# lyuchenyang/Macaw-LLM

Measured on NVIDIA H100. Metric: multimodal prefill tokens/sec (img+audio+text->LLaMA), higher is better.
Workload: dtype fp16

## Files before the change

### include/macaw_b200.h

```cpp
#ifndef MACAW_B200_H_
#define MACAW_B200_H_

#include <stdint.h>

#ifdef __cplusplus
extern "C" {
#endif

const char* mm_last_error(void);
int32_t mm_abi_version(void);
const char* mm_build_hash(void);
int64_t mm_launch_count(void);
void mm_launch_count_reset(void);
void mm_set_act_format(int32_t f16);
int32_t mm_get_act_format(void);

enum {
  MM_ACT_NONE = 0,
  MM_ACT_GELU = 1,
  MM_ACT_QUICK_GELU = 2,
  MM_ACT_SILU = 3
};
enum {
  MM_EPI_STD = 0,
  MM_EPI_SWIGLU = 1,
  MM_EPI_ROPE = 2
};

typedef struct mm_gemm_args {
  int32_t M, N, K, batch, batch2;
  const void* A;
  int64_t lda, a_bs, a_bs2;
  const void* B;
  int64_t ldb, b_bs, b_bs2;
  int32_t b_mn_major;
  void* C;
  int64_t ldc, c_bs, c_bs2;
  int32_t c_fp32;
  int32_t epi;
  int32_t act;
  float alpha;
  const void* bias;
  int64_t bias_bs;
  const float* row_scale;
  const void* residual;
  int64_t ldr, r_bs, r_bs2;
  int32_t res_row_mod;
  const float* rope_cos;
  const float* rope_sin;
  int32_t rope_T, rope_cols;
  const int32_t* rope_pos;
  int32_t c_trans;
  int32_t a_fp16, b_fp16;
  int32_t c_fp16;
  const float* bias_rs;
  const void* bias2;
  const float* bias2_rs;
  int32_t a_mn_major;
  float* sumsq_out;
  const float* rs_sumsq;
  int32_t rs_parts;
  float rs_eps;
  void* sk_workspace;
  int64_t sk_workspace_bytes;
} mm_gemm_args;

int32_t mm_gemm_fwd(const mm_gemm_args* args, void* stream);
enum {
  MM_GEMM_KERNEL_CONSUMER_EPILOGUE = 0,
  MM_GEMM_KERNEL_EPILOGUE_WARPGROUP = 1,
  MM_GEMM_KERNEL_TILE_PAIRS = 2
};
typedef struct mm_gemm_schedule {
  int32_t block_n;
  int32_t kernel;
  int32_t m_tiles, n_tiles, k_blocks;
  int64_t units;
  int32_t workers;
  int32_t grid;
  int32_t threads;
  int32_t waves;
  int32_t group_m;
  int32_t streamk_tiles;
  int32_t smem_bytes;
  int32_t vectorised_epilogue;
} mm_gemm_schedule;
int32_t mm_gemm_plan(const mm_gemm_args* args, mm_gemm_schedule* plan);
int32_t mm_gemm_streamk_mode(int32_t mode);
int32_t mm_gemm_overlap_mode(int32_t mode);
int64_t mm_gemm_streamk_workspace_bytes(void);

int32_t mm_splitk_reduce(const float* partial, int32_t splits, int32_t M, int32_t N, const void* bias, void* out,
                         int64_t ldo, int32_t out_fp16, void* stream);

typedef struct mm_attn_args {
  const void *q, *k, *v;
  void* out;
  int32_t B, H, Tq, Tk, head_dim;
  int64_t q_bs, q_ts, q_hs;
  int64_t k_bs, k_ts, k_hs;
  int64_t v_bs, v_ts, v_hs;
  int64_t o_bs, o_ts, o_hs;
  const int32_t* key_mask;
  int32_t causal;
  float scale;
  const int32_t* tk_dev;
} mm_attn_args;
int32_t mm_attn_fwd(const mm_attn_args* args, void* stream);

int32_t mm_rmsnorm_fwd(const void* x, const void* w, void* y, int32_t rows, int32_t cols, float eps, void* stream);
int32_t mm_rms_rstd(const void* x, float* rstd, int32_t rows, int32_t cols, float eps, void* stream);
int32_t mm_layernorm_fwd(const void* x, int64_t ldx, const void* w, const void* b, void* y, int64_t ldy, int32_t rows,
                         int32_t cols, float eps, void* stream);

int32_t mm_embed_gather(const void* table, int32_t vocab, int32_t dim, const int64_t* ids, int64_t n_ids, void* out,
                        int64_t ldo, void* stream);
int32_t mm_splice_prefix(const void* text, const void* prefix, void* dst, int32_t B, int32_t L, int32_t n_prefix,
                         int32_t E, const int64_t* mask_in, int64_t* mask_out, const int64_t* labels_in,
                         int64_t* labels_out, void* stream);
int32_t mm_patchify(const void* images, int32_t B, int32_t C, int32_t H, int32_t W, int32_t patch, void* out,
                    int64_t ldo, void* stream);
int32_t mm_transpose_pad(const void* x, int32_t B, int32_t C, int32_t T, int32_t pad, void* out, void* stream);
int32_t mm_add_rows(const void* x, int64_t ldx, const void* add, int64_t lda, int32_t add_rows, void* y, int64_t ldy,
                    int32_t rows, int32_t cols, void* stream);
int32_t mm_cast_bf16_f16(const void* x, int64_t ldx, void* y, int64_t ldy, int32_t rows, int32_t cols, void* stream);
int32_t mm_copy_rows(const void* x, int64_t ldx, void* y, int64_t ldy, int32_t rows, int32_t cols, void* stream);

typedef struct mm_align_args {
  const void* table;
  int32_t V, E;
  int64_t ldt;
  const void* qt;
  int32_t R;
  int64_t ldq;
  const float* row_bias;
  const float* extra;
  int64_t stat_stride;
  void* out;
  int64_t ldo;
  float* p_sum_real;
  float* p_extra;
  void* P;
  int64_t ldp;
  void* workspace;
  int32_t mode;
  float* inv_l;
} mm_align_args;
int32_t mm_align_fwd(const mm_align_args* args, void* stream);
int64_t mm_align_workspace_bytes(int32_t R, int32_t V);

int32_t mm_kv_append(const void* qkv, int64_t ld_qkv, int32_t B, int32_t T_new, int32_t E, void* cache, int32_t Tmax,
                     int32_t t0, const int32_t* t0_dev, void* stream);
int32_t mm_argmax_rows(const void* logits, int64_t ld, int32_t rows, int32_t V, int64_t* out, void* stream);
int32_t mm_sample_rows(const void* logits, int64_t ld, int32_t rows, int32_t V, uint32_t* seen, float repetition_penalty,
                       float temperature, int32_t top_k, float top_p, int32_t do_sample, const uint64_t* seed_dev,
                       const int32_t* step_dev, int64_t* out, void* stream);
enum { MM_THIN_RES = 0, MM_THIN_SWIGLU = 1, MM_THIN_QKV = 2 };
typedef struct mm_thin_args {
  const float* part;
  int32_t splits, N, M, ldp, mode;
  const float* row_scale;
  const float* rs_sumsq;
  int32_t rs_parts, rs_K;
  float rs_eps;
  const void* residual;
  int64_t ldr;
  void* out;
  int64_t ldo;
  float* sumsq_out;
  const float* rope_cos;
  const float* rope_sin;
  const int32_t* pos_dev;
  int32_t E;
  void* cache;
  int32_t Tmax, t0;
  const int32_t* t0_dev;
} mm_thin_args;
int32_t mm_thin_fused(const mm_thin_args* args, void* stream);
int32_t mm_rope_rows(void* x, int64_t ld, int32_t rows, int32_t rot_cols, const float* cos_t, const float* sin_t,
                     int32_t rope_T, const int32_t* pos_dev, void* stream);

int32_t mm_ce_loss(const void* logits, const int64_t* labels, int32_t B, int32_t T, int32_t V, float* loss_sum,
                   int32_t* n_valid, void* stream);

int32_t mm_rmsnorm_bwd_parts(int32_t rows);
int32_t mm_rmsnorm_bwd(const void* dy, const void* x, const float* rstd, const void* g, const void* dres, void* dx,
                       float* dg, float* dg_partials, int32_t rows, int32_t cols, void* stream);
int32_t mm_swiglu_fwd(const void* gate, const void* up, void* h, int64_t n, void* stream);
int32_t mm_swiglu_bwd(const void* dh, const void* gate, const void* up, void* dgate, void* dup, int64_t n, void* stream);
int32_t mm_attn_softmax_bwd(const float* S, const float* dP, void* P, void* dS, int32_t B, int32_t H, int32_t Tq,
                            int32_t Tk, int64_t ld, float scale, int32_t causal, const int32_t* key_mask, float p_drop,
                            const uint64_t* seed_dev, uint32_t sid, void* stream);
int32_t mm_attn_softmax_fwd(const float* S, void* P, int32_t B, int32_t H, int32_t Tq, int32_t Tk, int64_t ld, float scale,
                            int32_t causal, const int32_t* key_mask, float p_drop, const uint64_t* seed_dev, uint32_t sid,
                            void* stream);
int32_t mm_align_dropout_fwd(const void* P_unnorm_f16, void* Pm_f16, int64_t ldp, const float* inv_l, const float* p_extra,
                             float* rs, float* p_sum_real_d, float* p_extra_d, int32_t R, int32_t V, float p_drop,
                             const uint64_t* seed_dev, uint32_t sid, void* stream);
int32_t mm_dropout_mask(float* out, int64_t ld, int32_t rows, int32_t cols, float p_drop, const uint64_t* seed_dev,
                        uint32_t sid, void* stream);
int32_t mm_ce_bwd(const void* logits, const int64_t* labels, void* dlogits, int32_t B, int32_t T, int32_t V,
                  const int32_t* n_valid, float grad_scale, const float* grad_scale_dev, void* stream);
int32_t mm_embed_scatter_add(const void* dx, int64_t ldx, const int64_t* ids, int64_t n, int32_t dim, int32_t vocab,
                             void* dtable, void* stream);
int32_t mm_colsum(const void* x, int64_t ldx, int32_t rows, int32_t cols, float* out, void* stream);
int32_t mm_adamw(void* p, const void* g, float* master, float* m, float* v, int64_t n, float lr, float beta1, float beta2,
                 float eps, float weight_decay, int32_t step, const int32_t* step_dev, float grad_scale,
                 const float* grad_mult_dev, const int32_t* skip_dev, const float* lr_dev, void* stream);
int32_t mm_adamw_host(void* p, const void* g, float* master, float* m, float* v, int64_t n, float lr, float beta1,
                      float beta2, float eps, float weight_decay, int32_t step, const int32_t* step_dev, float grad_scale,
                      const float* grad_mult_dev, const int32_t* skip_dev, const float* lr_dev, void* stream);
int32_t mm_host_alloc(int64_t bytes, void** host_ptr, void** dev_ptr);
int32_t mm_host_free(void* host_ptr);

int32_t mm_grad_sumsq_parts(int64_t n);
int32_t mm_grad_sumsq(const void* g, int64_t n, int32_t fp16, float* out, float* partials, void* stream);
typedef struct mm_loss_scale_state {
  float scale;
  float inv_scale;
  int32_t cur_iter;
  int32_t last_overflow_iter;
  int32_t cur_hysteresis;
  int32_t skip;
  float grad_mult;
  int32_t skipped;
  int32_t step;
  float grad_norm;
  int32_t reserved[2];
} mm_loss_scale_state;
int32_t mm_loss_scale_update(mm_loss_scale_state* state, float* sumsq, float max_norm, int32_t dynamic, int32_t window,
                             int32_t hysteresis, float min_scale, void* stream);

int32_t mm_lr_schedule(const int32_t* step_dev, double base_lr, int32_t kind, int32_t warmup_steps, int32_t training_steps,
                       float* lr_out, void* stream);

int32_t mm_align_softmax_bwd(const float* G, int64_t ldg, const void* P_unnorm_f16, int64_t ldp, const float* inv_l,
                             const float* d_p_sum_real, const float* p_extra, const float* d_p_extra, float gscale,
                             void* P_bf16, void* dS_bf16, int64_t ldo, float* dstats, int32_t R, int32_t V, float p_drop,
                             const uint64_t* seed_dev, uint32_t sid, void* stream);
int32_t mm_head_weighted_colsum(const void* x, int64_t ldx, int32_t x_fp16, const float* w, int64_t w_stride, int32_t Nq,
                                int32_t E, int32_t head_dim, float* out, void* stream);
int32_t mm_window_gather_add(const void* dwin, int32_t B, int32_t N, int32_t C, int32_t Lq, int32_t kk, int32_t ss,
                             void* dfeats, void* stream);
int32_t mm_cast_f16_bf16(const void* x, int64_t ldx, void* y, int64_t ldy, int32_t rows, int32_t cols, void* stream);

#define MM_LORA_MAX 3
typedef struct mm_lora_args {
  int32_t n, M, K, N, r;
  float scaling, p_drop;
  const uint64_t* seed_dev;
  uint32_t sid[MM_LORA_MAX];
  const void* x;
  int64_t ldx;
  const void* A[MM_LORA_MAX];
  const void* B[MM_LORA_MAX];
  float* u[MM_LORA_MAX];
  void* y[MM_LORA_MAX];
  int64_t ldy;
  const float* rope_cos;
  const float* rope_sin;
  int32_t rope_T;
  float* g[MM_LORA_MAX];
  void* dA[MM_LORA_MAX];
  void* dB[MM_LORA_MAX];
  int32_t accumulate[MM_LORA_MAX];
  void* dx;
  int64_t lddx;
  float* workspace;
  int64_t workspace_bytes;
} mm_lora_args;
int32_t mm_lora_down(const mm_lora_args* args, void* stream);
int32_t mm_lora_up(const mm_lora_args* args, void* stream);
int32_t mm_lora_bwd_dy(const mm_lora_args* args, void* stream);
int32_t mm_lora_bwd_x(const mm_lora_args* args, void* stream);
int64_t mm_lora_workspace_bytes(const mm_lora_args* args, int32_t entry);

int32_t mm_nccl_unique_id(void* out128);
int32_t mm_nccl_init(const void* id128, int32_t world, int32_t rank);
int32_t mm_nccl_allreduce(void* buf, int64_t count, int32_t dtype, int32_t average, void* stream);
int32_t mm_nccl_destroy(void);

typedef struct mm_image_args {
  const void* src;
  int64_t ld;
  int32_t row0, n_rows;
  int32_t out_h, out_w;
  const int32_t* bounds_h;
  const int32_t* kk_h;
  int32_t ksize_h;
  const int32_t* bounds_v;
  const int32_t* kk_v;
  int32_t ksize_v;
  float mean[3], std[3];
  void* tmp;
  void* out;
  int32_t out_fp32;
  void* out_u8;
} mm_image_args;
int32_t mm_image_preprocess(const mm_image_args* args, void* stream);
int32_t mm_log_mel(const float* pcm, int32_t n_samples, const float* basisT, const float* mel, float* logspec,
                   void* max_scratch, void* out, int32_t out_fp32, void* stream);

#ifdef __cplusplus
}
#endif
#endif
```

### macaw-llm_b200/_lib.py

```python
from __future__ import annotations

import ctypes as C
import os

HERE = os.path.dirname(os.path.abspath(__file__))
LIB_PATH = os.path.join(HERE, "libmacaw_b200.so")

c_i32, c_i64, c_f32, c_vp, c_u32 = C.c_int32, C.c_int64, C.c_float, C.c_void_p, C.c_uint32


class GemmArgs(C.Structure):

    _fields_ = [
        ("M", c_i32), ("N", c_i32), ("K", c_i32), ("batch", c_i32), ("batch2", c_i32),
        ("A", c_vp), ("lda", c_i64), ("a_bs", c_i64), ("a_bs2", c_i64),
        ("B", c_vp), ("ldb", c_i64), ("b_bs", c_i64), ("b_bs2", c_i64), ("b_mn_major", c_i32),
        ("C", c_vp), ("ldc", c_i64), ("c_bs", c_i64), ("c_bs2", c_i64), ("c_fp32", c_i32),
        ("epi", c_i32), ("act", c_i32), ("alpha", c_f32),
        ("bias", c_vp), ("bias_bs", c_i64),
        ("row_scale", c_vp),
        ("residual", c_vp), ("ldr", c_i64), ("r_bs", c_i64), ("r_bs2", c_i64), ("res_row_mod", c_i32),
        ("rope_cos", c_vp), ("rope_sin", c_vp), ("rope_T", c_i32), ("rope_cols", c_i32), ("rope_pos", c_vp), ("c_trans", c_i32),
        ("a_fp16", c_i32), ("b_fp16", c_i32), ("c_fp16", c_i32),
        ("bias_rs", c_vp), ("bias2", c_vp), ("bias2_rs", c_vp), ("a_mn_major", c_i32),
        ("sumsq_out", c_vp), ("rs_sumsq", c_vp), ("rs_parts", c_i32), ("rs_eps", c_f32),
        ("sk_workspace", c_vp), ("sk_workspace_bytes", c_i64),
    ]


class GemmPlan(C.Structure):

    _fields_ = [("block_n", c_i32), ("kernel", c_i32), ("m_tiles", c_i32), ("n_tiles", c_i32), ("k_blocks", c_i32),
                ("units", c_i64), ("workers", c_i32), ("grid", c_i32), ("threads", c_i32), ("waves", c_i32),
                ("group_m", c_i32), ("streamk_tiles", c_i32), ("smem_bytes", c_i32), ("vectorised_epilogue", c_i32)]


class ThinArgs(C.Structure):
    _fields_ = [("part", c_vp), ("splits", c_i32), ("N", c_i32), ("M", c_i32), ("ldp", c_i32), ("mode", c_i32),
                ("row_scale", c_vp), ("rs_sumsq", c_vp), ("rs_parts", c_i32), ("rs_K", c_i32), ("rs_eps", c_f32),
                ("residual", c_vp), ("ldr", c_i64), ("out", c_vp), ("ldo", c_i64), ("sumsq_out", c_vp),
                ("rope_cos", c_vp), ("rope_sin", c_vp), ("pos_dev", c_vp), ("E", c_i32), ("cache", c_vp),
                ("Tmax", c_i32), ("t0", c_i32), ("t0_dev", c_vp)]


class AttnArgs(C.Structure):

    _fields_ = [
        ("q", c_vp), ("k", c_vp), ("v", c_vp), ("out", c_vp),
        ("B", c_i32), ("H", c_i32), ("Tq", c_i32), ("Tk", c_i32), ("head_dim", c_i32),
        ("q_bs", c_i64), ("q_ts", c_i64), ("q_hs", c_i64),
        ("k_bs", c_i64), ("k_ts", c_i64), ("k_hs", c_i64),
        ("v_bs", c_i64), ("v_ts", c_i64), ("v_hs", c_i64),
        ("o_bs", c_i64), ("o_ts", c_i64), ("o_hs", c_i64),
        ("key_mask", c_vp), ("causal", c_i32), ("scale", c_f32), ("tk_dev", c_vp),
    ]


class AlignArgs(C.Structure):

    _fields_ = [
        ("table", c_vp), ("V", c_i32), ("E", c_i32), ("ldt", c_i64),
        ("qt", c_vp), ("R", c_i32), ("ldq", c_i64),
        ("row_bias", c_vp), ("extra", c_vp), ("stat_stride", c_i64),
        ("out", c_vp), ("ldo", c_i64), ("p_sum_real", c_vp), ("p_extra", c_vp),
        ("P", c_vp), ("ldp", c_i64), ("workspace", c_vp), ("mode", c_i32), ("inv_l", c_vp),
    ]


LORA_MAX = 3


class LoraArgs(C.Structure):

    _fields_ = [
        ("n", c_i32), ("M", c_i32), ("K", c_i32), ("N", c_i32), ("r", c_i32), ("scaling", c_f32), ("p_drop", c_f32),
        ("seed_dev", c_vp), ("sid", c_u32 * LORA_MAX), ("x", c_vp), ("ldx", c_i64), ("A", c_vp * LORA_MAX),
        ("B", c_vp * LORA_MAX), ("u", c_vp * LORA_MAX), ("y", c_vp * LORA_MAX), ("ldy", c_i64), ("rope_cos", c_vp),
        ("rope_sin", c_vp), ("rope_T", c_i32), ("g", c_vp * LORA_MAX), ("dA", c_vp * LORA_MAX), ("dB", c_vp * LORA_MAX),
        ("accumulate", c_i32 * LORA_MAX), ("dx", c_vp), ("lddx", c_i64), ("workspace", c_vp), ("workspace_bytes", c_i64),
    ]


class LossScaleState(C.Structure):

    _fields_ = [("scale", c_f32), ("inv_scale", c_f32), ("cur_iter", c_i32), ("last_overflow_iter", c_i32),
                ("cur_hysteresis", c_i32), ("skip", c_i32), ("grad_mult", c_f32), ("skipped", c_i32), ("step", c_i32),
                ("grad_norm", c_f32), ("reserved", c_i32 * 2)]


class ImageArgs(C.Structure):

    _fields_ = [
        ("src", c_vp), ("ld", c_i64), ("row0", c_i32), ("n_rows", c_i32), ("out_h", c_i32), ("out_w", c_i32),
        ("bounds_h", c_vp), ("kk_h", c_vp), ("ksize_h", c_i32), ("bounds_v", c_vp), ("kk_v", c_vp), ("ksize_v", c_i32),
        ("mean", c_f32 * 3), ("std", c_f32 * 3), ("tmp", c_vp), ("out", c_vp), ("out_fp32", c_i32), ("out_u8", c_vp),
    ]


SIGNATURES = {
    "mm_last_error": (C.c_char_p, []),
    "mm_abi_version": (c_i32, []),
    "mm_build_hash": (C.c_char_p, []),
    "mm_launch_count": (c_i64, []),
    "mm_launch_count_reset": (None, []),
    "mm_set_act_format": (None, [c_i32]),
    "mm_get_act_format": (c_i32, []),
    "mm_gemm_fwd": (c_i32, [C.POINTER(GemmArgs), c_vp]),
    "mm_gemm_plan": (c_i32, [C.POINTER(GemmArgs), C.POINTER(GemmPlan)]),
    "mm_splitk_reduce": (c_i32, [c_vp, c_i32, c_i32, c_i32, c_vp, c_vp, c_i64, c_i32, c_vp]),
    "mm_attn_fwd": (c_i32, [C.POINTER(AttnArgs), c_vp]),
    "mm_rmsnorm_fwd": (c_i32, [c_vp, c_vp, c_vp, c_i32, c_i32, c_f32, c_vp]),
    "mm_rms_rstd": (c_i32, [c_vp, c_vp, c_i32, c_i32, c_f32, c_vp]),
    "mm_layernorm_fwd": (c_i32, [c_vp, c_i64, c_vp, c_vp, c_vp, c_i64, c_i32, c_i32, c_f32, c_vp]),
    "mm_embed_gather": (c_i32, [c_vp, c_i32, c_i32, c_vp, c_i64, c_vp, c_i64, c_vp]),
    "mm_splice_prefix": (c_i32, [c_vp, c_vp, c_vp, c_i32, c_i32, c_i32, c_i32, c_vp, c_vp, c_vp, c_vp, c_vp]),
    "mm_patchify": (c_i32, [c_vp, c_i32, c_i32, c_i32, c_i32, c_i32, c_vp, c_i64, c_vp]),
    "mm_transpose_pad": (c_i32, [c_vp, c_i32, c_i32, c_i32, c_i32, c_vp, c_vp]),
    "mm_add_rows": (c_i32, [c_vp, c_i64, c_vp, c_i64, c_i32, c_vp, c_i64, c_i32, c_i32, c_vp]),
    "mm_cast_bf16_f16": (c_i32, [c_vp, c_i64, c_vp, c_i64, c_i32, c_i32, c_vp]),
    "mm_copy_rows": (c_i32, [c_vp, c_i64, c_vp, c_i64, c_i32, c_i32, c_vp]),
    "mm_align_fwd": (c_i32, [C.POINTER(AlignArgs), c_vp]),
    "mm_align_workspace_bytes": (c_i64, [c_i32, c_i32]),
    "mm_kv_append": (c_i32, [c_vp, c_i64, c_i32, c_i32, c_i32, c_vp, c_i32, c_i32, c_vp, c_vp]),
    "mm_gemm_streamk_workspace_bytes": (c_i64, []),
    "mm_gemm_streamk_mode": (c_i32, [c_i32]),
    "mm_gemm_overlap_mode": (c_i32, [c_i32]),
    "mm_thin_fused": (c_i32, [C.POINTER(ThinArgs), c_vp]),
    "mm_argmax_rows": (c_i32, [c_vp, c_i64, c_i32, c_i32, c_vp, c_vp]),
    "mm_sample_rows": (c_i32, [c_vp, c_i64, c_i32, c_i32, c_vp, c_f32, c_f32, c_i32, c_f32, c_i32, c_vp, c_vp, c_vp, c_vp]),
    "mm_rope_rows": (c_i32, [c_vp, c_i64, c_i32, c_i32, c_vp, c_vp, c_i32, c_vp, c_vp]),
    "mm_rmsnorm_bwd": (c_i32, [c_vp, c_vp, c_vp, c_vp, c_vp, c_vp, c_vp, c_vp, c_i32, c_i32, c_vp]),
    "mm_rmsnorm_bwd_parts": (c_i32, [c_i32]),
    "mm_swiglu_fwd": (c_i32, [c_vp, c_vp, c_vp, c_i64, c_vp]),
    "mm_swiglu_bwd": (c_i32, [c_vp, c_vp, c_vp, c_vp, c_vp, c_i64, c_vp]),
    "mm_attn_softmax_bwd": (c_i32, [c_vp, c_vp, c_vp, c_vp, c_i32, c_i32, c_i32, c_i32, c_i64, c_f32, c_i32, c_vp, c_f32, c_vp,
                                    c_u32, c_vp]),
    "mm_attn_softmax_fwd": (c_i32, [c_vp, c_vp, c_i32, c_i32, c_i32, c_i32, c_i64, c_f32, c_i32, c_vp, c_f32, c_vp, c_u32, c_vp]),
    "mm_align_dropout_fwd": (c_i32, [c_vp, c_vp, c_i64, c_vp, c_vp, c_vp, c_vp, c_vp, c_i32, c_i32, c_f32, c_vp, c_u32, c_vp]),
    "mm_dropout_mask": (c_i32, [c_vp, c_i64, c_i32, c_i32, c_f32, c_vp, c_u32, c_vp]),
    "mm_ce_bwd": (c_i32, [c_vp, c_vp, c_vp, c_i32, c_i32, c_i32, c_vp, c_f32, c_vp, c_vp]),
    "mm_embed_scatter_add": (c_i32, [c_vp, c_i64, c_vp, c_i64, c_i32, c_i32, c_vp, c_vp]),
    "mm_colsum": (c_i32, [c_vp, c_i64, c_i32, c_i32, c_vp, c_vp]),
    "mm_adamw": (c_i32, [c_vp, c_vp, c_vp, c_vp, c_vp, c_i64, c_f32, c_f32, c_f32, c_f32, c_f32, c_i32, c_vp, c_f32, c_vp,
                         c_vp, c_vp, c_vp]),
    "mm_adamw_host": (c_i32, [c_vp, c_vp, c_vp, c_vp, c_vp, c_i64, c_f32, c_f32, c_f32, c_f32, c_f32, c_i32, c_vp, c_f32,
                              c_vp, c_vp, c_vp, c_vp]),
    "mm_lr_schedule": (c_i32, [c_vp, C.c_double, c_i32, c_i32, c_i32, c_vp, c_vp]),
    "mm_host_alloc": (c_i32, [c_i64, C.POINTER(c_vp), C.POINTER(c_vp)]),
    "mm_host_free": (c_i32, [c_vp]),
    "mm_grad_sumsq_parts": (c_i32, [c_i64]),
    "mm_grad_sumsq": (c_i32, [c_vp, c_i64, c_i32, c_vp, c_vp, c_vp]),
    "mm_loss_scale_update": (c_i32, [c_vp, c_vp, c_f32, c_i32, c_i32, c_i32, c_f32, c_vp]),
    "mm_image_preprocess": (c_i32, [C.POINTER(ImageArgs), c_vp]),
    "mm_log_mel": (c_i32, [c_vp, c_i32, c_vp, c_vp, c_vp, c_vp, c_vp, c_i32, c_vp]),
    "mm_align_softmax_bwd": (c_i32, [c_vp, c_i64, c_vp, c_i64, c_vp, c_vp, c_vp, c_vp, c_f32, c_vp, c_vp, c_i64, c_vp, c_i32,
                                     c_i32, c_f32, c_vp, c_u32, c_vp]),
    "mm_head_weighted_colsum": (c_i32, [c_vp, c_i64, c_i32, c_vp, c_i64, c_i32, c_i32, c_i32, c_vp, c_vp]),
    "mm_window_gather_add": (c_i32, [c_vp, c_i32, c_i32, c_i32, c_i32, c_i32, c_i32, c_vp, c_vp]),
    "mm_cast_f16_bf16": (c_i32, [c_vp, c_i64, c_vp, c_i64, c_i32, c_i32, c_vp]),
    "mm_nccl_unique_id": (c_i32, [c_vp]),
    "mm_nccl_init": (c_i32, [c_vp, c_i32, c_i32]),
    "mm_nccl_allreduce": (c_i32, [c_vp, c_i64, c_i32, c_i32, c_vp]),
    "mm_nccl_destroy": (c_i32, []),
    "mm_ce_loss": (c_i32, [c_vp, c_vp, c_i32, c_i32, c_i32, c_vp, c_vp, c_vp]),
    "mm_lora_down": (c_i32, [C.POINTER(LoraArgs), c_vp]),
    "mm_lora_up": (c_i32, [C.POINTER(LoraArgs), c_vp]),
    "mm_lora_bwd_dy": (c_i32, [C.POINTER(LoraArgs), c_vp]),
    "mm_lora_bwd_x": (c_i32, [C.POINTER(LoraArgs), c_vp]),
    "mm_lora_workspace_bytes": (c_i64, [C.POINTER(LoraArgs), c_i32]),
}

NULLABLE_BEFORE_STREAM = {"mm_adamw": 1, "mm_adamw_host": 1}

_lib = None
ABI_VERSION = 8


class _NullableBeforeStream:

    def __init__(self, fn, n_opt: int):
        self._fn, self._n_opt = fn, n_opt

    def __call__(self, *args):
        n = len(self._fn.argtypes)
        if n - self._n_opt <= len(args) < n:
            args = args[:-1] + (None,) * (n - len(args)) + args[-1:]
        return self._fn(*args)

    def __getattr__(self, name):
        return getattr(self._fn, name)


def load(build_if_missing: bool = True) -> C.CDLL:
    global _lib
    if _lib is not None:
        return _lib
    import importlib.util

    spec = importlib.util.spec_from_file_location("_macaw_b200_build", os.path.join(HERE, "build.py"))
    mod = importlib.util.module_from_spec(spec)
    spec.loader.exec_module(mod)
    want = mod.source_hash()
    if not os.path.exists(LIB_PATH) or mod.built_hash() != want:
        if not build_if_missing:
            raise RuntimeError(f"{LIB_PATH} is missing or older than csrc/; run `python macaw-llm_b200/build.py`")
        mod.build()
    lib = C.CDLL(LIB_PATH)
    for name, (res, args) in SIGNATURES.items():
        fn = getattr(lib, name)
        fn.restype = res
        fn.argtypes = args
        if name in NULLABLE_BEFORE_STREAM:
            setattr(lib, name, _NullableBeforeStream(fn, NULLABLE_BEFORE_STREAM[name]))
    got = lib.mm_build_hash().decode()
    if got != want or lib.mm_abi_version() != ABI_VERSION:
        raise RuntimeError(f"libmacaw_b200.so was built from other sources (library {got}, csrc {want}; ABI "
                           f"{lib.mm_abi_version()} vs {ABI_VERSION}): rebuild with `python macaw-llm_b200/build.py --force`")
    _lib = lib
    return lib


def last_error() -> str:
    return load().mm_last_error().decode("utf-8", "replace")
```

### macaw-llm_b200/csrc/attn_wgmma.cu

```cuda
#include "common.cuh"
#include "ptx.cuh"
#include "../../include/macaw_b200.h"

namespace mm {

struct FaParams {
  bf16* out;
  int B, H, Tq, Tk;
  long long o_bs, o_ts, o_hs;
  const int* key_mask;
  const int* tk_dev;
  int causal;
  float scale_log2;
  int hd;
};

constexpr int kFaMQ = 128;
constexpr int kFaKT = 64;
constexpr int kFaThreads = 288;

template <int HD>
__host__ __device__ constexpr size_t fa_smem_bytes() {
  return 1024 + (size_t)(HD / 64) * 16384 + 4 * (size_t)(HD / 64) * kFaKT * 128 + 256;
}

template <bool F16>
__device__ __forceinline__ void wgmma_s(float (&d)[kFaKT / 2], uint64_t a, uint64_t b, uint32_t acc) {
  wgmma_ss_n64<F16, 0, 0>(d, a, b, acc);
}
template <int HD, bool F16>
__device__ __forceinline__ void wgmma_pv(float (&d)[HD / 2], const uint32_t (&a)[4], uint64_t b) {
  if constexpr (HD == 128) wgmma_rs_n128<F16, 1>(d, a, b, 1u);
  else wgmma_rs_n64<F16, 1>(d, a, b, 1u);
}

template <int HD, bool F16>
__global__ void __launch_bounds__(kFaThreads, 1)
fa_wgmma_kernel(const __grid_constant__ CUtensorMap tmQ, const __grid_constant__ CUtensorMap tmK,
                const __grid_constant__ CUtensorMap tmV, const FaParams p) {
  constexpr int KB = HD / 64;
  constexpr uint32_t QBYTES = KB * 16384;
  constexpr uint32_t QB = KB * kFaKT * 128;
  constexpr int SB = kFaKT / 8;
  constexpr int NB = HD / 8;

  extern __shared__ uint8_t smem_raw[];
  uint8_t* smem = reinterpret_cast<uint8_t*>((reinterpret_cast<uintptr_t>(smem_raw) + 1023) & ~uintptr_t(1023));
  uint8_t* sQ = smem;
  uint8_t* sK = sQ + QBYTES;
  uint8_t* sV = sK + 2 * QB;
  uint64_t* bars = reinterpret_cast<uint64_t*>(sV + 2 * QB);
  uint64_t* bar_q = bars;
  uint64_t* bar_k = bars + 1;
  uint64_t* bar_v = bars + 3;
  uint64_t* bar_kfree = bars + 5;
  uint64_t* bar_vfree = bars + 7;

  const int warp = threadIdx.x >> 5, lane = threadIdx.x & 31;
  const int h = blockIdx.y, b = blockIdx.z;
  const int nq = (p.Tq + kFaMQ - 1) / kFaMQ;
  const int mt = p.causal ? nq - 1 - static_cast<int>(blockIdx.x) : static_cast<int>(blockIdx.x);
  const int q_base = p.causal ? p.Tq - nq * kFaMQ : 0;

  if (warp == 8 && elect_one()) {
    tma_prefetch_desc(&tmQ);
    tma_prefetch_desc(&tmK);
    tma_prefetch_desc(&tmV);
    mbar_init(bar_q, 1);
    for (int i = 0; i < 2; ++i) {
      mbar_init(&bar_k[i], 1);
      mbar_init(&bar_v[i], 1);
      mbar_init(&bar_kfree[i], 8);
      mbar_init(&bar_vfree[i], 8);
    }
    fence_mbar_init();
  }
  __syncthreads();
  griddep_launch();
  griddep_wait();
  int Tk = p.Tk;
  if (p.tk_dev != nullptr) Tk = min(*p.tk_dev, p.Tk);
  const int shift = Tk - p.Tq;
  int kv_end = Tk;
  if (p.causal) kv_end = min(Tk, q_base + mt * kFaMQ + kFaMQ + shift);
  const int n_tiles = kv_end > 0 ? (kv_end + kFaKT - 1) / kFaKT : 0;

  if (warp == 8) {
    if (n_tiles > 0 && elect_one()) {
      mbar_arrive_expect_tx(bar_q, QBYTES);
#pragma unroll
      for (int kb = 0; kb < KB; ++kb) tma_load_4d(&tmQ, bar_q, sQ + kb * 16384, kb * 64, q_base + mt * kFaMQ, h, b);
      for (int j = 0; j < n_tiles; ++j) {
        const int st = j & 1;
        const uint32_t par = ((j >> 1) - 1) & 1;
        if (j >= 2) mbar_wait(&bar_kfree[st], par);
        mbar_arrive_expect_tx(&bar_k[st], QB);
#pragma unroll
        for (int kb = 0; kb < KB; ++kb)
          tma_load_4d(&tmK, &bar_k[st], sK + st * QB + kb * (kFaKT * 128), kb * 64, j * kFaKT, h, b);
        if (j >= 2) mbar_wait(&bar_vfree[st], par);
        mbar_arrive_expect_tx(&bar_v[st], QB);
#pragma unroll
        for (int kb = 0; kb < KB; ++kb)
          tma_load_4d(&tmV, &bar_v[st], sV + st * QB + kb * (kFaKT * 128), kb * 64, j * kFaKT, h, b);
      }
    }
    return;
  }

  const int wg = warp >> 2;
  const int qrow0 = q_base + mt * kFaMQ + wg * 64 + (warp & 3) * 16 + (lane >> 2);
  const int* kmask = p.key_mask ? p.key_mask + static_cast<long long>(b) * p.Tk : nullptr;
  float o[HD / 2];
#pragma unroll
  for (int i = 0; i < HD / 2; ++i) o[i] = 0.f;
  float row_m[2] = {-INFINITY, -INFINITY};
  float row_l[2] = {0.f, 0.f};
  if (n_tiles > 0) mbar_wait(bar_q, 0);
  const uint32_t q_addr = smem_u32(sQ) + wg * 8192;

  for (int j = 0; j < n_tiles; ++j) {
    const int st = j & 1;
    const uint32_t par = (j >> 1) & 1;
    float s[kFaKT / 2];
#pragma unroll
    for (int i = 0; i < kFaKT / 2; ++i) s[i] = 0.f;
    mbar_wait(&bar_k[st], par);
    const uint32_t k_addr = smem_u32(sK + st * QB);
    wgmma_fence();
#pragma unroll
    for (int k = 0; k < HD / 16; ++k) {
      if (k * 16 >= p.hd) break;
      wgmma_s<F16>(s, make_sdesc_sw128(q_addr + (k >> 2) * 16384 + (k & 3) * 32, 16, 1024),
                   make_sdesc_sw128(k_addr + (k >> 2) * (kFaKT * 128) + (k & 3) * 32, 16, 1024), 1u);
    }
    wgmma_commit();
    wgmma_wait<0>();
    fence_regs(s);
    __syncwarp();
    if (lane == 0) mbar_arrive(&bar_kfree[st]);

    const int key0 = j * kFaKT + (lane & 3) * 2;
    const bool full = kmask == nullptr && j * kFaKT + kFaKT <= Tk &&
                      (!p.causal || j * kFaKT + kFaKT - 1 <= qrow0 + shift);
    float mx[2] = {-INFINITY, -INFINITY};
    if (full) {
#pragma unroll
      for (int i = 0; i < kFaKT / 2; ++i) {
        s[i] *= p.scale_log2;
        mx[(i >> 1) & 1] = fmaxf(mx[(i >> 1) & 1], s[i]);
      }
    } else {
#pragma unroll
      for (int nb = 0; nb < SB; ++nb) {
#pragma unroll
        for (int e = 0; e < 4; ++e) {
          const int key = key0 + nb * 8 + (e & 1);
          const int qrow = qrow0 + (e >> 1) * 8;
          bool ok = key < Tk;
          if (p.causal) ok = ok && (key <= qrow + shift);
          if (kmask != nullptr && ok) ok = __ldg(kmask + key) != 0;
          const float v = ok ? s[4 * nb + e] * p.scale_log2 : -INFINITY;
          s[4 * nb + e] = v;
          mx[e >> 1] = fmaxf(mx[e >> 1], v);
        }
      }
    }
    float corr[2];
#pragma unroll
    for (int r = 0; r < 2; ++r) {
      mx[r] = fmaxf(mx[r], __shfl_xor_sync(0xffffffffu, mx[r], 1));
      mx[r] = fmaxf(mx[r], __shfl_xor_sync(0xffffffffu, mx[r], 2));
      const float m_new = fmaxf(row_m[r], mx[r]);
      const float m_safe = (m_new == -INFINITY) ? 0.f : m_new;
      corr[r] = exp2f(row_m[r] - m_safe);
      row_m[r] = m_new;
      mx[r] = m_safe;
    }
    float ls[2] = {0.f, 0.f};
#pragma unroll
    for (int i = 0; i < kFaKT / 2; ++i) {
      const float pv = exp2f(s[i] - mx[(i >> 1) & 1]);
      s[i] = pv;
      ls[(i >> 1) & 1] += pv;
    }
#pragma unroll
    for (int r = 0; r < 2; ++r) row_l[r] = row_l[r] * corr[r] + ls[r];
#pragma unroll
    for (int nb = 0; nb < NB; ++nb) {
      o[4 * nb] *= corr[0];
      o[4 * nb + 1] *= corr[0];
      o[4 * nb + 2] *= corr[1];
      o[4 * nb + 3] *= corr[1];
    }

    uint32_t pa[kFaKT / 16][4];
#pragma unroll
    for (int kc = 0; kc < kFaKT / 16; ++kc) {
      pa[kc][0] = pack2<F16>(s[8 * kc + 0], s[8 * kc + 1]);
      pa[kc][1] = pack2<F16>(s[8 * kc + 2], s[8 * kc + 3]);
      pa[kc][2] = pack2<F16>(s[8 * kc + 4], s[8 * kc + 5]);
      pa[kc][3] = pack2<F16>(s[8 * kc + 6], s[8 * kc + 7]);
    }
    mbar_wait(&bar_v[st], par);
    const uint32_t v_addr = smem_u32(sV + st * QB);
    wgmma_fence();
#pragma unroll
    for (int kc = 0; kc < kFaKT / 16; ++kc)
      wgmma_pv<HD, F16>(o, pa[kc], make_sdesc_sw128(v_addr + kc * 2048, kFaKT * 128, 1024));
    wgmma_commit();
    wgmma_wait<0>();
    fence_regs(o);
    __syncwarp();
    if (lane == 0) mbar_arrive(&bar_vfree[st]);
  }

#pragma unroll
  for (int r = 0; r < 2; ++r) {
    float l = row_l[r];
    l += __shfl_xor_sync(0xffffffffu, l, 1);
    l += __shfl_xor_sync(0xffffffffu, l, 2);
    row_l[r] = l > 0.f ? 1.0f / l : 0.f;
  }
  bf16* og = p.out + static_cast<long long>(b) * p.o_bs + static_cast<long long>(h) * p.o_hs;
#pragma unroll
  for (int r = 0; r < 2; ++r) {
    const int qrow = qrow0 + 8 * r;
    if (qrow < 0 || qrow >= p.Tq) continue;
    uint32_t* orow = reinterpret_cast<uint32_t*>(og + static_cast<long long>(qrow) * p.o_ts);
#pragma unroll
    for (int nb = 0; nb < NB; ++nb)
      if (nb * 8 < p.hd) orow[nb * 4 + (lane & 3)] = pack2<F16>(o[4 * nb + 2 * r] * row_l[r], o[4 * nb + 2 * r + 1] * row_l[r]);
  }
}

typedef CUresult (*EncodeTiledFn2)(CUtensorMap*, CUtensorMapDataType, cuuint32_t, void*, const cuuint64_t*,
                                   const cuuint64_t*, const cuuint32_t*, const cuuint32_t*, CUtensorMapInterleave,
                                   CUtensorMapSwizzle, CUtensorMapL2promotion, CUtensorMapFloatOOBfill);

static int fa_make_map(CUtensorMap* m, const void* ptr, int hd, int T, int H, int B, int64_t ts, int64_t hs, int64_t bs,
                       uint32_t box_rows) {
  static EncodeTiledFn2 fn = nullptr;
  if (fn == nullptr) {
    void* f = nullptr;
    cudaDriverEntryPointQueryResult q;
    if (cudaGetDriverEntryPoint("cuTensorMapEncodeTiled", &f, cudaEnableDefault, &q) == cudaSuccess &&
        q == cudaDriverEntryPointSuccess)
      fn = reinterpret_cast<EncodeTiledFn2>(f);
  }
  if (fn == nullptr) {
    set_error("cuTensorMapEncodeTiled entry point unavailable");
    return 1;
  }
  if (hs <= 0) hs = static_cast<int64_t>(hd);
  if (bs <= 0) bs = static_cast<int64_t>(T) * ts;
  cuuint64_t dims[4] = {static_cast<cuuint64_t>(hd), static_cast<cuuint64_t>(T), static_cast<cuuint64_t>(H),
                        static_cast<cuuint64_t>(B)};
  cuuint64_t strides[3] = {static_cast<cuuint64_t>(ts) * 2, static_cast<cuuint64_t>(hs) * 2,
                           static_cast<cuuint64_t>(bs) * 2};
  cuuint32_t box[4] = {64, box_rows, 1, 1};
  cuuint32_t estr[4] = {1, 1, 1, 1};
  CUresult r = fn(m, CU_TENSOR_MAP_DATA_TYPE_BFLOAT16, 4, const_cast<void*>(ptr), dims, strides, box, estr,
                  CU_TENSOR_MAP_INTERLEAVE_NONE, CU_TENSOR_MAP_SWIZZLE_128B, CU_TENSOR_MAP_L2_PROMOTION_L2_256B,
                  CU_TENSOR_MAP_FLOAT_OOB_FILL_NONE);
  if (r != CUDA_SUCCESS) {
    set_error("mm_attn_fwd: cuTensorMapEncodeTiled failed (%d) hd=%d T=%d H=%d B=%d ts=%lld hs=%lld bs=%lld",
              static_cast<int>(r), hd, T, H, B, (long long)ts, (long long)hs, (long long)bs);
    return 1;
  }
  return 0;
}

template <int HD, bool F16>
static int launch_fa(const mm_attn_args* a, cudaStream_t st) {
  static bool attr_set[kMaxDevices] = {};
  constexpr size_t smem = fa_smem_bytes<HD>();
  if (int rc = ensure_smem_attr(fa_wgmma_kernel<HD, F16>, smem, attr_set, "mm_attn_fwd")) return rc;
  CUtensorMap tq, tk, tv;
  const int hd = a->head_dim;
  if (fa_make_map(&tq, a->q, hd, a->Tq, a->H, a->B, a->q_ts, a->q_hs, a->q_bs, kFaMQ)) return 1;
  if (fa_make_map(&tk, a->k, hd, a->Tk, a->H, a->B, a->k_ts, a->k_hs, a->k_bs, kFaKT)) return 1;
  if (fa_make_map(&tv, a->v, hd, a->Tk, a->H, a->B, a->v_ts, a->v_hs, a->v_bs, kFaKT)) return 1;
  FaParams p;
  p.hd = hd;
  p.out = reinterpret_cast<bf16*>(a->out);
  p.B = a->B; p.H = a->H; p.Tq = a->Tq; p.Tk = a->Tk;
  p.o_bs = a->o_bs; p.o_ts = a->o_ts; p.o_hs = a->o_hs;
  p.key_mask = a->key_mask;
  p.tk_dev = a->tk_dev;
  p.causal = a->causal;
  p.scale_log2 = a->scale * 1.4426950408889634f;
  const int nq = (a->Tq + kFaMQ - 1) / kFaMQ;
  dim3 grid(nq, a->H, a->B);
  cudaError_t e = launch_kernel(fa_wgmma_kernel<HD, F16>, grid, dim3(kFaThreads), smem, st, 1, tq, tk, tv, p);
  if (e != cudaSuccess) {
    set_error("mm_attn_fwd: launch failed: %s", cudaGetErrorString(e));
    return 2;
  }
  return check_launch("mm_attn_fwd(wgmma)");
}

}
using namespace mm;

extern "C" int32_t mm_attn_fwd(const mm_attn_args* a, void* stream) {
  MM_REQUIRE(a && a->q && a->k && a->v && a->out, "mm_attn_fwd: null argument");
  MM_REQUIRE(a->B > 0 && a->H > 0 && a->Tq > 0 && a->Tk > 0, "mm_attn_fwd: bad shape");
  MM_REQUIRE(a->head_dim == 64 || a->head_dim == 96 || a->head_dim == 128, "mm_attn_fwd: head_dim %d unsupported",
             a->head_dim);
  MM_REQUIRE(a->scale > 0.f, "mm_attn_fwd: scale must be positive");
  const int64_t strides[] = {a->q_bs, a->q_ts, a->q_hs, a->k_bs, a->k_ts, a->k_hs,
                             a->v_bs, a->v_ts, a->v_hs, a->o_bs, a->o_ts, a->o_hs};
  for (int64_t s : strides) MM_REQUIRE(s % 8 == 0, "mm_attn_fwd: strides must be multiples of 8 elements");
  MM_REQUIRE(((uintptr_t)a->q % 16 == 0) && ((uintptr_t)a->k % 16 == 0) && ((uintptr_t)a->v % 16 == 0) &&
                 ((uintptr_t)a->out % 16 == 0),
             "mm_attn_fwd: pointers must be 16-byte aligned");
  cudaStream_t st = reinterpret_cast<cudaStream_t>(stream);
  if (act_f16()) return a->head_dim == 64 ? launch_fa<64, true>(a, st) : launch_fa<128, true>(a, st);
  return a->head_dim == 64 ? launch_fa<64, false>(a, st) : launch_fa<128, false>(a, st);
}
```

Before: 38350.

## Add persistent pipelined flash-attention schedule with overlapped QK/PV and ping-pong option

Adds a persistent-grid flash-attention variant. A producer warp streams K/V tiles through a 4-stage TMA ring and double-buffers Q, and the consumer warpgroups overlap the next QK wgmma with the current PV wgmma and softmax. Work items are grouped by batch-head, reversed for causal, and distributed serpentine across SMs. A serial path that unrolls the QK loop without an early break is kept for non-causal, unmasked calls. Mode is selectable via env/API (default 1); the pipelined path uses more shared memory and adds complexity, and may trail the serial kernel on short sequences.

New measurement: 39400, median of 6. 1.03x the previous value.

```diff
diff --git a/include/macaw_b200.h b/include/macaw_b200.h
--- a/include/macaw_b200.h
+++ b/include/macaw_b200.h
@@ -107,6 +107,7 @@
   const int32_t* tk_dev;
 } mm_attn_args;
 int32_t mm_attn_fwd(const mm_attn_args* args, void* stream);
+int32_t mm_attn_schedule_mode(int32_t mode);
 
 int32_t mm_rmsnorm_fwd(const void* x, const void* w, void* y, int32_t rows, int32_t cols, float eps, void* stream);
 int32_t mm_rms_rstd(const void* x, float* rstd, int32_t rows, int32_t cols, float eps, void* stream);
diff --git a/macaw-llm_b200/_lib.py b/macaw-llm_b200/_lib.py
--- a/macaw-llm_b200/_lib.py
+++ b/macaw-llm_b200/_lib.py
@@ -125,6 +125,7 @@
     "mm_gemm_streamk_workspace_bytes": (c_i64, []),
     "mm_gemm_streamk_mode": (c_i32, [c_i32]),
     "mm_gemm_overlap_mode": (c_i32, [c_i32]),
+    "mm_attn_schedule_mode": (c_i32, [c_i32]),
     "mm_thin_fused": (c_i32, [C.POINTER(ThinArgs), c_vp]),
     "mm_argmax_rows": (c_i32, [c_vp, c_i64, c_i32, c_i32, c_vp, c_vp]),
     "mm_sample_rows": (c_i32, [c_vp, c_i64, c_i32, c_i32, c_vp, c_f32, c_f32, c_i32, c_f32, c_i32, c_vp, c_vp, c_vp, c_vp]),
diff --git a/macaw-llm_b200/csrc/attn_wgmma.cu b/macaw-llm_b200/csrc/attn_wgmma.cu
--- a/macaw-llm_b200/csrc/attn_wgmma.cu
+++ b/macaw-llm_b200/csrc/attn_wgmma.cu
@@ -13,6 +13,7 @@
   int causal;
   float scale_log2;
   int hd;
+  int gbh;
 };
 
 constexpr int kFaMQ = 128;
@@ -34,10 +35,17 @@
   else wgmma_rs_n64<F16, 1>(d, a, b, 1u);
 }
 
-template <int HD, bool F16>
-__global__ void __launch_bounds__(kFaThreads, 1)
-fa_wgmma_kernel(const __grid_constant__ CUtensorMap tmQ, const __grid_constant__ CUtensorMap tmK,
-                const __grid_constant__ CUtensorMap tmV, const FaParams p) {
+template <int KSTEPS, bool F16>
+__device__ __forceinline__ void fa_qk(float (&s)[kFaKT / 2], uint32_t q_addr, uint32_t k_addr) {
+#pragma unroll
+  for (int k = 0; k < KSTEPS; ++k)
+    wgmma_s<F16>(s, make_sdesc_sw128(q_addr + (k >> 2) * 16384 + (k & 3) * 32, 16, 1024),
+                 make_sdesc_sw128(k_addr + (k >> 2) * (kFaKT * 128) + (k & 3) * 32, 16, 1024), 1u);
+}
+
+template <int HD, bool F16, bool UNBROKEN_QK>
+__device__ __forceinline__ void fa_serial(const CUtensorMap& tmQ, const CUtensorMap& tmK, const CUtensorMap& tmV,
+                                          const FaParams& p) {
   constexpr int KB = HD / 64;
   constexpr uint32_t QBYTES = KB * 16384;
   constexpr uint32_t QB = KB * kFaKT * 128;
@@ -128,11 +136,18 @@
     mbar_wait(&bar_k[st], par);
     const uint32_t k_addr = smem_u32(sK + st * QB);
     wgmma_fence();
-#pragma unroll
-    for (int k = 0; k < HD / 16; ++k) {
-      if (k * 16 >= p.hd) break;
-      wgmma_s<F16>(s, make_sdesc_sw128(q_addr + (k >> 2) * 16384 + (k & 3) * 32, 16, 1024),
-                   make_sdesc_sw128(k_addr + (k >> 2) * (kFaKT * 128) + (k & 3) * 32, 16, 1024), 1u);
+    if constexpr (UNBROKEN_QK) {
+      if (HD == 128 && p.hd == 96)
+        fa_qk<6, F16>(s, q_addr, k_addr);
+      else
+        fa_qk<HD / 16, F16>(s, q_addr, k_addr);
+    } else {
+#pragma unroll
+      for (int k = 0; k < HD / 16; ++k) {
+        if (k * 16 >= p.hd) break;
+        wgmma_s<F16>(s, make_sdesc_sw128(q_addr + (k >> 2) * 16384 + (k & 3) * 32, 16, 1024),
+                     make_sdesc_sw128(k_addr + (k >> 2) * (kFaKT * 128) + (k & 3) * 32, 16, 1024), 1u);
+      }
     }
     wgmma_commit();
     wgmma_wait<0>();
@@ -232,6 +247,315 @@
     for (int nb = 0; nb < NB; ++nb)
       if (nb * 8 < p.hd) orow[nb * 4 + (lane & 3)] = pack2<F16>(o[4 * nb + 2 * r] * row_l[r], o[4 * nb + 2 * r + 1] * row_l[r]);
   }
+}
+
+constexpr int kFaStages = 4;
+
+template <int HD>
+__host__ __device__ constexpr size_t fa_pipe_smem_bytes() {
+  return 1024 + 2 * (size_t)(HD / 64) * 16384 + 2 * kFaStages * (size_t)(HD / 64) * kFaKT * 128 + 256;
+}
+
+struct FaItem {
+  int mt, h, b;
+};
+__device__ __forceinline__ int fa_item_index(int round, int n_items) {
+  const int G = static_cast<int>(gridDim.x), c = static_cast<int>(blockIdx.x);
+  const int it = round * G + ((round & 1) ? G - 1 - c : c);
+  return it < n_items ? it : -1;
+}
+__device__ __forceinline__ FaItem fa_item(int it, const FaParams& p, int nq) {
+  const int per = p.gbh * nq;
+  const int g = it / per, r = it - g * per;
+  const int gb = min(p.gbh, p.B * p.H - g * p.gbh);
+  const int t = r / gb;
+  const int bh = g * p.gbh + (r - t * gb);
+  FaItem x;
+  x.mt = p.causal ? nq - 1 - t : t;
+  x.h = bh % p.H;
+  x.b = bh / p.H;
+  return x;
+}
+
+__device__ __forceinline__ void fa_turn_wait(int wg) { asm volatile("bar.sync %0, 256;" ::"r"(1 + wg) : "memory"); }
+__device__ __forceinline__ void fa_turn_pass(int wg) { asm volatile("bar.arrive %0, 256;" ::"r"(2 - wg) : "memory"); }
+
+template <int HD, bool F16, bool PINGPONG>
+__device__ __forceinline__ void fa_pipelined(const CUtensorMap& tmQ, const CUtensorMap& tmK, const CUtensorMap& tmV,
+                                             const FaParams& p) {
+  constexpr int KB = HD / 64;
+  constexpr uint32_t QBYTES = KB * 16384;
+  constexpr uint32_t QB = KB * kFaKT * 128;
+  constexpr int SB = kFaKT / 8;
+  constexpr int NB = HD / 8;
+  constexpr int NS = kFaStages;
+
+  extern __shared__ uint8_t smem_raw[];
+  uint8_t* smem = reinterpret_cast<uint8_t*>((reinterpret_cast<uintptr_t>(smem_raw) + 1023) & ~uintptr_t(1023));
+  uint8_t* sQ = smem;
+  uint8_t* sK = sQ + 2 * QBYTES;
+  uint8_t* sV = sK + NS * QB;
+  uint64_t* bars = reinterpret_cast<uint64_t*>(sV + NS * QB);
+  uint64_t* bar_q = bars;
+  uint64_t* bar_qfree = bars + 2;
+  uint64_t* bar_k = bars + 4;
+  uint64_t* bar_v = bar_k + NS;
+  uint64_t* bar_kfree = bar_v + NS;
+  uint64_t* bar_vfree = bar_kfree + NS;
+  uint64_t* kbits = bar_vfree + NS;
+
+  const int warp = threadIdx.x >> 5, lane = threadIdx.x & 31;
+  const int nq = (p.Tq + kFaMQ - 1) / kFaMQ;
+  const int n_items = nq * p.B * p.H;
+  const int q_base = p.causal ? p.Tq - nq * kFaMQ : 0;
+
+  if (warp == 8 && elect_one()) {
+    tma_prefetch_desc(&tmQ);
+    tma_prefetch_desc(&tmK);
+    tma_prefetch_desc(&tmV);
+    for (int i = 0; i < 2; ++i) {
+      mbar_init(&bar_q[i], 1);
+      mbar_init(&bar_qfree[i], 8);
+    }
+    for (int i = 0; i < NS; ++i) {
+      mbar_init(&bar_k[i], 1);
+      mbar_init(&bar_v[i], 1);
+      mbar_init(&bar_kfree[i], 8);
+      mbar_init(&bar_vfree[i], 8);
+    }
+    fence_mbar_init();
+  }
+  __syncthreads();
+  griddep_launch();
+  griddep_wait();
+  int Tk = p.Tk;
+  if (p.tk_dev != nullptr) Tk = min(*p.tk_dev, p.Tk);
+  const int shift = Tk - p.Tq;
+  auto tiles_of = [&](int mt) {
+    int kv_end = Tk;
+    if (p.causal) kv_end = min(Tk, q_base + mt * kFaMQ + kFaMQ + shift);
+    return kv_end > 0 ? (kv_end + kFaKT - 1) / kFaKT : 0;
+  };
+
+  if (warp == 8) {
+    uint32_t g = 0;
+    uint32_t qn = 0;
+    for (int round = 0;; ++round) {
+      const int it = fa_item_index(round, n_items);
+      if (it < 0) break;
+      const FaItem x = fa_item(it, p, nq);
+      const int n_tiles = tiles_of(x.mt);
+      if (n_tiles == 0) continue;
+      if (lane == 0) {
+        const int qb = qn & 1;
+        if (qn >= 2) mbar_wait(&bar_qfree[qb], ((qn >> 1) - 1) & 1);
+        mbar_arrive_expect_tx(&bar_q[qb], QBYTES);
+#pragma unroll
+        for (int kb = 0; kb < KB; ++kb)
+          tma_load_4d(&tmQ, &bar_q[qb], sQ + qb * QBYTES + kb * 16384, kb * 64, q_base + x.mt * kFaMQ, x.h, x.b);
+      }
+      ++qn;
+      const int* km = p.key_mask ? p.key_mask + static_cast<long long>(x.b) * p.Tk : nullptr;
+      for (int j = 0; j < n_tiles; ++j, ++g) {
+        const int st = g % NS;
+        const uint32_t use = g / NS;
+        const int key = j * kFaKT + lane;
+        const bool lo = key < Tk && (km == nullptr || __ldg(km + key) != 0);
+        const bool hi = key + 32 < Tk && (km == nullptr || __ldg(km + key + 32) != 0);
+        const uint32_t wlo = __ballot_sync(0xffffffffu, lo), whi = __ballot_sync(0xffffffffu, hi);
+        if (lane == 0) {
+          if (use > 0) mbar_wait(&bar_kfree[st], (use - 1) & 1);
+          kbits[st] = (static_cast<uint64_t>(whi) << 32) | wlo;
+          mbar_arrive_expect_tx(&bar_k[st], QB);
+#pragma unroll
+          for (int kb = 0; kb < KB; ++kb)
+            tma_load_4d(&tmK, &bar_k[st], sK + st * QB + kb * (kFaKT * 128), kb * 64, j * kFaKT, x.h, x.b);
+          if (use > 0) mbar_wait(&bar_vfree[st], (use - 1) & 1);
+          mbar_arrive_expect_tx(&bar_v[st], QB);
+#pragma unroll
+          for (int kb = 0; kb < KB; ++kb)
+            tma_load_4d(&tmV, &bar_v[st], sV + st * QB + kb * (kFaKT * 128), kb * 64, j * kFaKT, x.h, x.b);
+        }
+        __syncwarp();
+      }
+    }
+    return;
+  }
+
+  const int wg = warp >> 2;
+  if (PINGPONG && wg == 1) fa_turn_pass(wg);
+  uint32_t g = 0, qn = 0;
+  for (int round = 0;; ++round) {
+    const int it = fa_item_index(round, n_items);
+    if (it < 0) break;
+    const FaItem x = fa_item(it, p, nq);
+    const int n_tiles = tiles_of(x.mt);
+    const int wrow0 = q_base + x.mt * kFaMQ + wg * 64 + (warp & 3) * 16;
+    const int qrow0 = wrow0 + (lane >> 2);
+    const uint32_t q_addr = smem_u32(sQ) + (qn & 1) * QBYTES + wg * 8192;
+    float o[HD / 2];
+#pragma unroll
+    for (int i = 0; i < HD / 2; ++i) o[i] = 0.f;
+    float row_m[2] = {-INFINITY, -INFINITY};
+    float row_l[2] = {0.f, 0.f};
+    float s[kFaKT / 2];
+    uint32_t pa[kFaKT / 16][4];
+
+    auto issue_s = [&](uint32_t gj) {
+      const int st = gj % NS;
+      mbar_wait(&bar_k[st], (gj / NS) & 1);
+      const uint32_t k_addr = smem_u32(sK + st * QB);
+#pragma unroll
+      for (int i = 0; i < kFaKT / 2; ++i) s[i] = 0.f;
+      wgmma_fence();
+      if (HD == 128 && p.hd == 96)
+        fa_qk<6, F16>(s, q_addr, k_addr);
+      else
+        fa_qk<HD / 16, F16>(s, q_addr, k_addr);
+      wgmma_commit();
+    };
+    auto issue_pv = [&](uint32_t gj) {
+      const int st = gj % NS;
+      mbar_wait(&bar_v[st], (gj / NS) & 1);
+      const uint32_t v_addr = smem_u32(sV + st * QB);
+      wgmma_fence();
+#pragma unroll
+      for (int kc = 0; kc < kFaKT / 16; ++kc)
+        wgmma_pv<HD, F16>(o, pa[kc], make_sdesc_sw128(v_addr + kc * 2048, kFaKT * 128, 1024));
+      wgmma_commit();
+    };
+    auto softmax = [&](int j, uint32_t gj, float (&corr)[2]) {
+      fence_regs(s);
+      const int st = gj % NS;
+      const uint64_t bits = kbits[st];
+      __syncwarp();
+      if (lane == 0) {
+        mbar_arrive(&bar_kfree[st]);
+        if (j == n_tiles - 1) mbar_arrive(&bar_qfree[(qn - 1) & 1]);
+      }
+      const bool full = bits == ~0ull && (!p.causal || j * kFaKT + kFaKT - 1 <= wrow0 + shift);
+      float mx[2] = {-INFINITY, -INFINITY};
+      if (full) {
+#pragma unroll
+        for (int i = 0; i < kFaKT / 2; ++i) {
+          s[i] *= p.scale_log2;
+          mx[(i >> 1) & 1] = fmaxf(mx[(i >> 1) & 1], s[i]);
+        }
+      } else {
+        const int key0 = j * kFaKT + (lane & 3) * 2;
+#pragma unroll
+        for (int nb = 0; nb < SB; ++nb) {
+#pragma unroll
+          for (int e = 0; e < 4; ++e) {
+            const int kk = (lane & 3) * 2 + nb * 8 + (e & 1);
+            bool ok = (bits >> kk) & 1;
+            if (p.causal) ok = ok && (key0 + nb * 8 + (e & 1) <= qrow0 + (e >> 1) * 8 + shift);
+            const float v = ok ? s[4 * nb + e] * p.scale_log2 : -INFINITY;
+            s[4 * nb + e] = v;
+            mx[e >> 1] = fmaxf(mx[e >> 1], v);
+          }
+        }
+      }
+#pragma unroll
+      for (int r = 0; r < 2; ++r) {
+        mx[r] = fmaxf(mx[r], __shfl_xor_sync(0xffffffffu, mx[r], 1));
+        mx[r] = fmaxf(mx[r], __shfl_xor_sync(0xffffffffu, mx[r], 2));
+        const float m_new = fmaxf(row_m[r], mx[r]);
+        const float m_safe = (m_new == -INFINITY) ? 0.f : m_new;
+        corr[r] = exp2f(row_m[r] - m_safe);
+        row_m[r] = m_new;
+        mx[r] = m_safe;
+      }
+      float ls[2] = {0.f, 0.f};
+#pragma unroll
+      for (int i = 0; i < kFaKT / 2; ++i) {
+        const float pv = exp2f(s[i] - mx[(i >> 1) & 1]);
+        s[i] = pv;
+        ls[(i >> 1) & 1] += pv;
+      }
+#pragma unroll
+      for (int r = 0; r < 2; ++r) row_l[r] = row_l[r] * corr[r] + ls[r];
+    };
+    auto rescale_pack = [&](const float (&corr)[2]) {
+#pragma unroll
+      for (int nb = 0; nb < NB; ++nb) {
+        o[4 * nb] *= corr[0];
+        o[4 * nb + 1] *= corr[0];
+        o[4 * nb + 2] *= corr[1];
+        o[4 * nb + 3] *= corr[1];
+      }
+#pragma unroll
+      for (int kc = 0; kc < kFaKT / 16; ++kc) {
+        pa[kc][0] = pack2<F16>(s[8 * kc + 0], s[8 * kc + 1]);
+        pa[kc][1] = pack2<F16>(s[8 * kc + 2], s[8 * kc + 3]);
+        pa[kc][2] = pack2<F16>(s[8 * kc + 4], s[8 * kc + 5]);
+        pa[kc][3] = pack2<F16>(s[8 * kc + 6], s[8 * kc + 7]);
+      }
+    };
+    auto release_v = [&](uint32_t gj) {
+      fence_regs(o);
+      __syncwarp();
+      if (lane == 0) mbar_arrive(&bar_vfree[gj % NS]);
+    };
+
+    if (n_tiles > 0) {
+      mbar_wait(&bar_q[qn & 1], (qn >> 1) & 1);
+      ++qn;
+      float corr[2];
+      if (PINGPONG) fa_turn_wait(wg);
+      issue_s(g);
+      if (PINGPONG) fa_turn_pass(wg);
+      wgmma_wait<0>();
+      softmax(0, g, corr);
+      rescale_pack(corr);
+      for (int j = 1; j < n_tiles; ++j) {
+        if (PINGPONG) fa_turn_wait(wg);
+        issue_s(g + j);
+        issue_pv(g + j - 1);
+        if (PINGPONG) fa_turn_pass(wg);
+        wgmma_wait<1>();
+        softmax(j, g + j, corr);
+        wgmma_wait<0>();
+        release_v(g + j - 1);
+        rescale_pack(corr);
+      }
+      if (PINGPONG) fa_turn_wait(wg);
+      issue_pv(g + n_tiles - 1);
+      if (PINGPONG) fa_turn_pass(wg);
+      wgmma_wait<0>();
+      release_v(g + n_tiles - 1);
+      g += n_tiles;
+    }
+
+#pragma unroll
+    for (int r = 0; r < 2; ++r) {
+      float l = row_l[r];
+      l += __shfl_xor_sync(0xffffffffu, l, 1);
+      l += __shfl_xor_sync(0xffffffffu, l, 2);
+      row_l[r] = l > 0.f ? 1.0f / l : 0.f;
+    }
+    bf16* og = p.out + static_cast<long long>(x.b) * p.o_bs + static_cast<long long>(x.h) * p.o_hs;
+#pragma unroll
+    for (int r = 0; r < 2; ++r) {
+      const int qrow = qrow0 + 8 * r;
+      if (qrow < 0 || qrow >= p.Tq) continue;
+      uint32_t* orow = reinterpret_cast<uint32_t*>(og + static_cast<long long>(qrow) * p.o_ts);
+#pragma unroll
+      for (int nb = 0; nb < NB; ++nb)
+        if (nb * 8 < p.hd) orow[nb * 4 + (lane & 3)] = pack2<F16>(o[4 * nb + 2 * r] * row_l[r], o[4 * nb + 2 * r + 1] * row_l[r]);
+    }
+  }
+  if (PINGPONG && wg == 0) fa_turn_wait(wg);
+}
+
+template <int HD, bool F16, int SCHED>
+__global__ void __launch_bounds__(kFaThreads, 1)
+fa_wgmma_kernel(const __grid_constant__ CUtensorMap tmQ, const __grid_constant__ CUtensorMap tmK,
+                const __grid_constant__ CUtensorMap tmV, const FaParams p) {
+  if constexpr (SCHED == 0 || SCHED == 3)
+    fa_serial<HD, F16, SCHED == 3>(tmQ, tmK, tmV, p);
+  else
+    fa_pipelined<HD, F16, SCHED == 2>(tmQ, tmK, tmV, p);
 }
 
 typedef CUresult (*EncodeTiledFn2)(CUtensorMap*, CUtensorMapDataType, cuuint32_t, void*, const cuuint64_t*,
@@ -271,11 +595,17 @@
   return 0;
 }
 
-template <int HD, bool F16>
+static int& attn_schedule_mode() {
+  static int mode = []() { const char* e = getenv("MACAW_B200_ATTN_SCHEDULE"); const int v = e ? atoi(e) : 1; return v < 0 || v > 3 ? 1 : v; }();
+  return mode;
+}
+
+template <int HD, bool F16, int SCHED>
 static int launch_fa(const mm_attn_args* a, cudaStream_t st) {
   static bool attr_set[kMaxDevices] = {};
-  constexpr size_t smem = fa_smem_bytes<HD>();
-  if (int rc = ensure_smem_attr(fa_wgmma_kernel<HD, F16>, smem, attr_set, "mm_attn_fwd")) return rc;
+  constexpr bool serial = SCHED == 0 || SCHED == 3;
+  constexpr size_t smem = serial ? fa_smem_bytes<HD>() : fa_pipe_smem_bytes<HD>();
+  if (int rc = ensure_smem_attr(fa_wgmma_kernel<HD, F16, SCHED>, smem, attr_set, "mm_attn_fwd")) return rc;
   CUtensorMap tq, tk, tv;
   const int hd = a->head_dim;
   if (fa_make_map(&tq, a->q, hd, a->Tq, a->H, a->B, a->q_ts, a->q_hs, a->q_bs, kFaMQ)) return 1;
@@ -292,12 +622,27 @@
   p.scale_log2 = a->scale * 1.4426950408889634f;
   const int nq = (a->Tq + kFaMQ - 1) / kFaMQ;
   dim3 grid(nq, a->H, a->B);
-  cudaError_t e = launch_kernel(fa_wgmma_kernel<HD, F16>, grid, dim3(kFaThreads), smem, st, 1, tq, tk, tv, p);
+  p.gbh = 1;
+  if (!serial) {
+    const long long items = static_cast<long long>(nq) * a->H * a->B;
+    const int ctas = static_cast<int>(std::min<long long>(num_sms(), items));
+    p.gbh = std::max(1, ctas / nq);
+    grid = dim3(ctas, 1, 1);
+  }
+  cudaError_t e = launch_kernel(fa_wgmma_kernel<HD, F16, SCHED>, grid, dim3(kFaThreads), smem, st, 1, tq, tk, tv, p);
   if (e != cudaSuccess) {
     set_error("mm_attn_fwd: launch failed: %s", cudaGetErrorString(e));
     return 2;
   }
   return check_launch("mm_attn_fwd(wgmma)");
+}
+
+template <int HD, bool F16>
+static int launch_fa_mode(const mm_attn_args* a, cudaStream_t st) {
+  const int mode = attn_schedule_mode();
+  if (mode == 0) return launch_fa<HD, F16, 0>(a, st);
+  if (mode == 1 && !a->causal && a->key_mask == nullptr) return launch_fa<HD, F16, 3>(a, st);
+  return mode == 3 ? launch_fa<HD, F16, 2>(a, st) : launch_fa<HD, F16, 1>(a, st);
 }
 
 }
@@ -316,6 +661,12 @@
                  ((uintptr_t)a->out % 16 == 0),
              "mm_attn_fwd: pointers must be 16-byte aligned");
   cudaStream_t st = reinterpret_cast<cudaStream_t>(stream);
-  if (act_f16()) return a->head_dim == 64 ? launch_fa<64, true>(a, st) : launch_fa<128, true>(a, st);
-  return a->head_dim == 64 ? launch_fa<64, false>(a, st) : launch_fa<128, false>(a, st);
-}
+  if (act_f16()) return a->head_dim == 64 ? launch_fa_mode<64, true>(a, st) : launch_fa_mode<128, true>(a, st);
+  return a->head_dim == 64 ? launch_fa_mode<64, false>(a, st) : launch_fa_mode<128, false>(a, st);
+}
+
+extern "C" int32_t mm_attn_schedule_mode(int32_t mode) {
+  const int prev = attn_schedule_mode();
+  if (mode >= 0 && mode <= 3) attn_schedule_mode() = mode;
+  return prev;
+}
```
